# lucidrains/vit-pytorch

Hardware: NVIDIA H100
Metric: images/sec ViT-B/16 224^2 bf16 fwd (higher is better)
Workload: dtype bf16

## Files before the change

### vit_pytorch_b200/build.py

```python
from __future__ import annotations

import concurrent.futures as cf
import os
import shutil
import subprocess
import sys
from pathlib import Path

PKG = Path(__file__).resolve().parent
CSRC = PKG / "csrc"
LIBDIR = PKG / "lib"
OBJDIR = PKG / "lib" / "obj"
LIB = LIBDIR / "libb200vit.so"

NVCC_FLAGS = [
    "-gencode", "arch=compute_90a,code=sm_90a",
    "-std=c++17", "-O3", "-lineinfo",
    "-Xcompiler", "-fPIC",
    "--expt-relaxed-constexpr",
]


def _nvcc() -> str:
    nvcc = shutil.which("nvcc") or "/usr/local/cuda/bin/nvcc"
    if not os.path.exists(nvcc):
        raise RuntimeError("nvcc not found; libb200vit.so must be prebuilt in-tree")
    return nvcc


def sources() -> list[Path]:
    return sorted(CSRC.glob("*.cu"))


def needs_build() -> bool:
    if not LIB.exists():
        return True
    t = LIB.stat().st_mtime
    deps = list(CSRC.glob("*.cu")) + list(CSRC.glob("*.cuh")) + list(CSRC.glob("*.h")) + \
        [PKG.parent / "include" / "b200vit.h"]
    return any(d.stat().st_mtime > t for d in deps)


def _compile(src: Path, verbose: bool) -> Path:
    obj = OBJDIR / (src.stem + ".o")
    cmd = [_nvcc(), *NVCC_FLAGS, "-c", str(src), "-o", str(obj)]
    if verbose:
        cmd.insert(1, "-Xptxas")
        cmd.insert(2, "-v")
    r = subprocess.run(cmd, capture_output=True, text=True)
    if r.returncode != 0:
        raise RuntimeError(f"nvcc failed for {src.name}:\n{r.stdout}\n{r.stderr}")
    if verbose:
        print(r.stderr)
    return obj


def build(force: bool = False, verbose: bool = False) -> Path:
    if not force and not needs_build():
        return LIB
    OBJDIR.mkdir(parents=True, exist_ok=True)
    srcs = sources()
    with cf.ThreadPoolExecutor(max_workers=min(8, len(srcs))) as ex:
        objs = list(ex.map(lambda s: _compile(s, verbose), srcs))
    cmd = [_nvcc(), "-shared", "-gencode", "arch=compute_90a,code=sm_90a", "-o", str(LIB), *map(str, objs)]
    r = subprocess.run(cmd, capture_output=True, text=True)
    if r.returncode != 0:
        raise RuntimeError(f"link failed:\n{r.stdout}\n{r.stderr}")
    return LIB


if __name__ == "__main__":
    p = build(force="--force" in sys.argv, verbose="-v" in sys.argv)
    print(p)
```

### vit_pytorch_b200/csrc/gemm.cu

```cuda
#include "common.cuh"
#include "host_util.h"

namespace b200 {

constexpr int BLOCK_M = 128;
constexpr int BLOCK_K = 64;
constexpr int WGMMA_K = 16;
constexpr int NUM_THREADS = 384;
constexpr int NUM_CONSUMERS = 256;

struct GemmParams {
  int M, N, K;
  int num_m_tiles, num_n_tiles, num_k_blocks;
  int flags;
  __nv_bfloat16* out_bf16;
  float* out_f32;
  long long ldo;
  const float* bias;
  const float* ln_sums;
  int ln_parts;
  int stats_parts;
  int stats_width;
  float ln_inv_dim;
  float ln_eps;
  const float* col_s;
  float* stats_out;
  int rows_per_tile;
  int patch;
  int patch_ght;
  int patch_tiles_per_img;
  int patch_C;
};

template <int BLOCK_N, int STAGES, bool PATCH = false, bool RES = false, bool TMA_OUT = false>
struct GemmSmem {
  static constexpr bool BIAS_ONLY = RES && TMA_OUT && BLOCK_N == 256;
  static constexpr bool RING_SLABS = BIAS_ONLY;
  static constexpr int BUF_SLABS = RING_SLABS ? 0 : BLOCK_N / 64;
  static constexpr int A_SLAB = PATCH ? BLOCK_M * 32 : BLOCK_M * BLOCK_K * 2;
  static constexpr int A_BYTES = PATCH ? 4 * A_SLAB : A_SLAB;
  static constexpr int B_BYTES = BLOCK_N * BLOCK_K * 2;
  static constexpr int STAGE_BYTES = A_BYTES + B_BYTES;
  static constexpr int RES_BOX = BLOCK_M * 32 * 4;
  static constexpr int RES_SLAB = 2 * RES_BOX;
  static constexpr int RES_OFFSET = STAGES * STAGE_BYTES;
  static constexpr int OUT_BOX = 64 * 64 * 2;
  static constexpr int OUT_OFFSET = RES_OFFSET + (RES && !RING_SLABS ? 2 * RES_SLAB : 0);
  static constexpr int OUT_BYTES = !TMA_OUT ? 0 : RES ? 2 * OUT_BOX : BLOCK_M * BLOCK_N * 2;
  static constexpr int VEC_OFFSET = OUT_OFFSET + OUT_BYTES;
  static constexpr int VEC_BYTES = (BIAS_ONLY ? BLOCK_N : 2 * BLOCK_N + 2 * BLOCK_M) * 4;
  static constexpr int VEC_BUFS = BIAS_ONLY ? 1 : 2;
  static constexpr int BAR_OFFSET = VEC_OFFSET + VEC_BUFS * VEC_BYTES;
  static constexpr int TOTAL = BAR_OFFSET + (2 * STAGES + 8) * 8;
  static constexpr int DYN_BYTES = TOTAL + 1024;
};

__device__ __forceinline__ void warpgroup_sync(int c) { asm volatile("bar.sync %0, 128;" ::"r"(c + 1) : "memory"); }

template <int BLOCK_N, int STAGES, bool PATCH, bool RES, bool TMA_OUT, bool SIG = false, int EPI = -1>
__global__ void __launch_bounds__(NUM_THREADS, 1)
gemm_bf16_kernel(const __grid_constant__ CUtensorMap tmA, const __grid_constant__ CUtensorMap tmB,
                 const __grid_constant__ CUtensorMap tmR, const __grid_constant__ CUtensorMap tmO,
                 const __grid_constant__ CUtensorMap tmF, const GemmParams p) {
  static_assert(!(TMA_OUT && PATCH), "patch tiles have fewer than 128 rows: a 64-row box would overwrite the next one");
  static_assert(EPI < 0 || (TMA_OUT && !SIG), "compiled flag sets are for the TMA-store epilogue");
  using L = GemmSmem<BLOCK_N, STAGES, PATCH, RES, TMA_OUT>;
  constexpr int NACC = BLOCK_N / 2;
  constexpr int CHUNKS = BLOCK_N / 64;

  extern __shared__ uint8_t smem_raw[];
  uint8_t* smem = smem_raw + ((1024u - (smem_u32(smem_raw) & 1023u)) & 1023u);
  uint64_t* full_bar = reinterpret_cast<uint64_t*>(smem + L::BAR_OFFSET);
  uint64_t* empty_bar = full_bar + STAGES;
  uint64_t* res_full = empty_bar + STAGES;
  uint64_t* res_empty = res_full + 2;
  uint64_t* vec_full = res_empty + 2;
  uint64_t* vec_empty = vec_full + 2;

  const int wg = threadIdx.x >> 7;
  const int num_tiles = p.num_m_tiles * p.num_n_tiles;

  if (threadIdx.x == 0) {
    tma_prefetch_desc(&tmA);
    tma_prefetch_desc(&tmB);
    if (RES) tma_prefetch_desc(&tmR);
    if (TMA_OUT && p.out_bf16) tma_prefetch_desc(&tmO);
    if (TMA_OUT && RES && p.out_f32) tma_prefetch_desc(&tmF);
    for (int s = 0; s < STAGES; ++s) {
      mbar_init(&full_bar[s], 1);
      mbar_init(&empty_bar[s], 2);
    }
    for (int s = 0; s < 2; ++s) {
      mbar_init(&res_full[s], 1);
      mbar_init(&res_empty[s], TMA_OUT ? 2 : NUM_CONSUMERS);
      mbar_init(&vec_full[s], 64);
      mbar_init(&vec_empty[s], NUM_CONSUMERS);
    }
    fence_mbar_init();
  }
  __syncthreads();

  if (wg == 0) {
    setmaxnreg_dec<40>();
    if (threadIdx.x == 0) {
      int stage = 0;
      uint32_t phase = 0;
      for (int tile = blockIdx.x; tile < num_tiles; tile += gridDim.x) {
        const int m_blk = tile / p.num_n_tiles;
        const int n_blk = tile % p.num_n_tiles;
        for (int kb = 0; kb < p.num_k_blocks; ++kb) {
          mbar_wait(&empty_bar[stage], phase ^ 1);
          uint8_t* sa = smem + stage * L::STAGE_BYTES;
          uint8_t* sb = sa + L::A_BYTES;
          if (PATCH) {
            const int img = m_blk / p.patch_tiles_per_img, tin = m_blk % p.patch_tiles_per_img;
            mbar_arrive_expect_tx(&full_bar[stage], p.rows_per_tile * 128 + L::B_BYTES);
#pragma unroll
            for (int j = 0; j < 4; ++j)
              tma_load_5d(sa + j * L::A_SLAB, &tmA, &full_bar[stage], 0, 0, tin * p.patch_ght, (kb & 3) * 4 + j,
                          img * p.patch_C + (kb >> 2));
          } else {
            mbar_arrive_expect_tx(&full_bar[stage], L::STAGE_BYTES);
            tma_load_2d(sa, &tmA, &full_bar[stage], kb * BLOCK_K, m_blk * BLOCK_M);
          }
          tma_load_2d(sb, &tmB, &full_bar[stage], kb * BLOCK_K, n_blk * BLOCK_N);
          if (++stage == STAGES) {
            stage = 0;
            phase ^= 1;
          }
        }
        if (L::RING_SLABS) {
          const int n0 = n_blk * BLOCK_N;
          const int nslab = min(BLOCK_N / 64, (p.N - n0 + 63) / 64);
          for (int q = L::BUF_SLABS; q < nslab; ++q) {
            mbar_wait(&empty_bar[stage], phase ^ 1);
            const int c0 = n0 + 64 * q;
            const int nbox = c0 + 32 < p.N ? 2 : 1;
            mbar_arrive_expect_tx(&full_bar[stage], nbox * L::RES_BOX);
            uint8_t* slab = smem + stage * L::STAGE_BYTES;
            for (int b = 0; b < nbox; ++b)
              tma_load_2d(slab + b * L::RES_BOX, &tmR, &full_bar[stage], c0 + 32 * b, m_blk * BLOCK_M);
            if (++stage == STAGES) {
              stage = 0;
              phase ^= 1;
            }
          }
        }
      }
    } else if (RES && threadIdx.x == 32) {
      int it = 0;
      for (int tile = blockIdx.x; tile < num_tiles; tile += gridDim.x) {
        const int n0 = (tile % p.num_n_tiles) * BLOCK_N;
        const int m0 = (tile / p.num_n_tiles) * BLOCK_M;
        const int nslab = min(L::BUF_SLABS, (p.N - n0 + 63) / 64);
        for (int q = 0; q < nslab; ++q, ++it) {
          const int buf = it & 1;
          mbar_wait(&res_empty[buf], ((it >> 1) & 1) ^ 1);
          const int c0 = n0 + 64 * q;
          const int nbox = c0 + 32 < p.N ? 2 : 1;
          mbar_arrive_expect_tx(&res_full[buf], nbox * L::RES_BOX);
          uint8_t* slab = smem + L::RES_OFFSET + buf * L::RES_SLAB;
          for (int b = 0; b < nbox; ++b) tma_load_2d(slab + b * L::RES_BOX, &tmR, &res_full[buf], c0 + 32 * b, m0);
        }
      }
    } else if ((threadIdx.x >> 5) >= 2) {
      const int lane = threadIdx.x & 31;
      const bool vec_warp = (threadIdx.x >> 5) == 2;
      int it = 0;
      for (int tile = blockIdx.x; tile < num_tiles; tile += gridDim.x, ++it) {
        const int m_blk = tile / p.num_n_tiles;
        const int n0 = (tile % p.num_n_tiles) * BLOCK_N;
        const int vb = it % L::VEC_BUFS;
        mbar_wait(&vec_empty[vb], ((it / L::VEC_BUFS) & 1) ^ 1);
        float* vbias = reinterpret_cast<float*>(smem + L::VEC_OFFSET + vb * L::VEC_BYTES);
        float* vcs = vbias + BLOCK_N;
        float2* vln = reinterpret_cast<float2*>(vcs + BLOCK_N);
        if (vec_warp) {
#pragma unroll
          for (int i = lane; i < BLOCK_N; i += 32) {
            const int col = n0 + i;
            vbias[i] = (p.flags & B200VIT_EPI_BIAS) && col < p.N ? p.bias[col] : 0.f;
            if (!L::BIAS_ONLY) vcs[i] = (p.flags & B200VIT_EPI_LNFOLD) && col < p.N ? p.col_s[col] : 0.f;
          }
        } else if (!L::BIAS_ONLY && (p.flags & B200VIT_EPI_LNFOLD)) {
          float s1[BLOCK_M / 32], s2[BLOCK_M / 32];
          bool ok[BLOCK_M / 32];
#pragma unroll
          for (int k = 0; k < BLOCK_M / 32; ++k) {
            const int tr = lane + 32 * k;
            ok[k] = m_blk * p.rows_per_tile + tr < p.M && tr < p.rows_per_tile;
            s1[k] = s2[k] = 0.f;
          }
#pragma unroll 1
          for (int i = 0; i < p.ln_parts; ++i)
#pragma unroll
            for (int k = 0; k < BLOCK_M / 32; ++k)
              if (ok[k]) {
                const size_t row = (size_t)m_blk * p.rows_per_tile + lane + 32 * k;
                const float2 ss = *reinterpret_cast<const float2*>(p.ln_sums + 2 * (row * p.ln_parts + i));
                s1[k] += ss.x;
                s2[k] += ss.y;
              }
#pragma unroll
          for (int k = 0; k < BLOCK_M / 32; ++k) vln[lane + 32 * k] = make_float2(s1[k], s2[k]);
        }
        mbar_arrive(&vec_full[vb]);
      }
    }
    return;
  }

  setmaxnreg_inc<232>();
  const int c = wg - 1;
  const int t = threadIdx.x & 127;
  const int warp = t >> 5, lane = t & 31;
  const int flags = EPI >= 0 ? EPI : L::BIAS_ONLY ? p.flags & ~B200VIT_EPI_LNFOLD : p.flags;
  const bool vec_ok = (p.ldo & 1) == 0;
  int stage = 0;
  uint32_t phase = 0;
  int slab_it = 0;
  int pend_slab = -1;
  uint8_t* const stg_wg = smem + L::OUT_OFFSET + c * (RES ? L::OUT_BOX : 64 * BLOCK_N * 2);
  float acc[NACC];

  for (int tile = blockIdx.x, it = 0; tile < num_tiles; tile += gridDim.x, ++it) {
    const int m_blk = tile / p.num_n_tiles;
    const int n_blk = tile % p.num_n_tiles;

    int prev_stage = -1;
    for (int kb = 0; kb < p.num_k_blocks; ++kb) {
      mbar_wait(&full_bar[stage], phase);
      const uint32_t sa = smem_u32(smem + stage * L::STAGE_BYTES);
      const uint32_t sb = sa + L::A_BYTES;
      const uint64_t bdesc = make_wgmma_desc(sb, 1024, WGMMA_SW128);
      wgmma_fence();
#pragma unroll
      for (int k = 0; k < BLOCK_K / WGMMA_K; ++k) {
        const uint64_t ad = PATCH ? make_wgmma_desc(sa + k * L::A_SLAB + c * 64 * 32, 256, WGMMA_SW32)
                                  : make_wgmma_desc(sa + c * 64 * 128, 1024, WGMMA_SW128) + 2 * k;
        if constexpr (BLOCK_N == 256) wgmma_m64n256k16(acc, ad, bdesc + 2 * k, (kb | k) != 0);
        else wgmma_m64n128k16(acc, ad, bdesc + 2 * k, (kb | k) != 0);
      }
      wgmma_commit();
      if (TMA_OUT && kb == 0 && t == 0) {
        tma_store_wait_read<0>();
        if (RES && pend_slab >= 0) mbar_arrive(&empty_bar[pend_slab]);
        pend_slab = -1;
      }
      wgmma_wait<1>();
      if (prev_stage >= 0 && t == 0) mbar_arrive(&empty_bar[prev_stage]);
      prev_stage = stage;
      if (++stage == STAGES) {
        stage = 0;
        phase ^= 1;
      }
    }
    wgmma_wait<0>();
    fence_regs(acc);
    if (t == 0) mbar_arrive(&empty_bar[prev_stage]);
    if (TMA_OUT && !RES) warpgroup_sync(c);

    const int tr0 = c * 64 + warp * 16 + (lane >> 2);
    const int vb = it % L::VEC_BUFS;
    mbar_wait(&vec_full[vb], (it / L::VEC_BUFS) & 1);
    const float* vbias = reinterpret_cast<const float*>(smem + L::VEC_OFFSET + vb * L::VEC_BYTES);
    const float* vcs = vbias + BLOCK_N;
    const float2* vln = reinterpret_cast<const float2*>(vcs + BLOCK_N);
    float mu[2] = {0.f, 0.f}, rstd[2] = {1.f, 1.f};
    int row[2];
    bool row_ok[2];
#pragma unroll
    for (int h = 0; h < 2; ++h) {
      const int tr = tr0 + 8 * h;
      row[h] = m_blk * p.rows_per_tile + tr;
      row_ok[h] = row[h] < p.M && tr < p.rows_per_tile;
      if ((flags & B200VIT_EPI_LNFOLD) && row_ok[h]) {
        const float2 ss = vln[tr];
        const float s1 = ss.x, s2 = ss.y;
        mu[h] = s1 * p.ln_inv_dim;
        const float var = fmaxf(s2 * p.ln_inv_dim - mu[h] * mu[h], 0.f);
        rstd[h] = rsqrtf(var + p.ln_eps);
      }
    }
    float st_sum[2][CHUNKS], st_sq[2][CHUNKS];
#pragma unroll
    for (int q = 0; q < CHUNKS; ++q) st_sum[0][q] = st_sum[1][q] = st_sq[0][q] = st_sq[1][q] = 0.f;

    const int n0 = n_blk * BLOCK_N;
    const int nslab = RES ? min(CHUNKS, (p.N - n0 + 63) / 64) : 0;
    const int res_off = tr0 * 128 + (lane & 1) * 8;
    const int res_xor = ((lane & 3) >> 1) ^ (lane >> 2);
    const int stg_off = (tr0 - 64 * c) * 128 + 4 * (lane & 3);
    constexpr bool GUARD = EPI < 0 || RES;
#pragma unroll
    for (int j = 0; j < BLOCK_N / 8; ++j) {
      const int pc = 8 * j + 2 * (lane & 3);
      const int col = n0 + pc;
      const bool ring_slab = L::RING_SLABS && j / 8 >= L::BUF_SLABS;
      if (RES && j % 8 == 0 && j / 8 < nslab) {
        if (ring_slab) mbar_wait(&full_bar[stage], phase);
        else mbar_wait(&res_full[slab_it & 1], (slab_it >> 1) & 1);
      }
      uint8_t* const slab_base =
          smem + (ring_slab ? stage * L::STAGE_BYTES : L::RES_OFFSET + (slab_it & 1) * L::RES_SLAB);
      uint8_t* slab = slab_base + ((j % 8) / 4) * L::RES_BOX + res_off;
      uint8_t* stg = stg_wg + (RES ? 0 : (j / 8) * L::OUT_BOX) + stg_off + (((j % 8) ^ (lane >> 2)) << 4);
      const bool pair = vec_ok && col + 1 < p.N;
      float b0 = 0.f, b1 = 0.f, s0 = 0.f, s1 = 0.f;
      if (flags & B200VIT_EPI_BIAS) {
        const float2 bb = *reinterpret_cast<const float2*>(vbias + pc);
        b0 = bb.x;
        b1 = bb.y;
      }
      if (flags & B200VIT_EPI_LNFOLD) {
        const float2 ss = *reinterpret_cast<const float2*>(vcs + pc);
        s0 = ss.x;
        s1 = ss.y;
      }
#pragma unroll
      for (int h = 0; h < 2; ++h) {
        if (GUARD && (!row_ok[h] || col >= p.N)) continue;
        float v0 = acc[4 * j + 2 * h], v1 = acc[4 * j + 2 * h + 1];
        if (flags & (B200VIT_EPI_LNFOLD | B200VIT_EPI_BIAS)) {
          const bool fold = (flags & B200VIT_EPI_LNFOLD) != 0;
          const float k = -rstd[h] * mu[h];
          const float c0 = fold ? fmaf(k, s0, b0) : b0, c1 = fold ? fmaf(k, s1, b1) : b1;
          const float rs = fold ? rstd[h] : 1.0f;
          v0 = fmaf(v0, rs, c0);
          v1 = fmaf(v1, rs, c1);
        }
        if (flags & B200VIT_EPI_GELU) gelu_erf2(v0, v1);
        if (flags & B200VIT_EPI_HARDSWISH) {
          v0 = v0 * fminf(fmaxf(v0 + 3.0f, 0.0f), 6.0f) * (1.0f / 6.0f);
          v1 = v1 * fminf(fmaxf(v1 + 3.0f, 0.0f), 6.0f) * (1.0f / 6.0f);
        }
        if (SIG && (flags & (B200VIT_EPI_SILU | B200VIT_EPI_SIGMOID))) {
          const float g0 = fast_rcp(1.0f + fast_ex2(-1.4426950408889634f * v0));
          const float g1 = fast_rcp(1.0f + fast_ex2(-1.4426950408889634f * v1));
          const bool silu = (flags & B200VIT_EPI_SILU) != 0;
          v0 = silu ? v0 * g0 : g0;
          v1 = silu ? v1 * g1 : g1;
        }
        const size_t o = (size_t)row[h] * p.ldo + col;
        float2* rp = reinterpret_cast<float2*>(slab + h * 8 * 128 + ((((j % 4) * 2) ^ res_xor) << 4));
        float2 rr = make_float2(0.f, 0.f);
        if (RES) rr = *rp;
        float r0 = 0.f, r1 = 0.f;
        if (TMA_OUT) {
          if (RES) {
            v0 += rr.x;
            v1 += rr.y;
            *rp = make_float2(v0, v1);
          }
          const uint32_t pk = pack_bf16x2(v0, v1);
          if (!RES) *reinterpret_cast<uint32_t*>(stg + h * 8 * 128) = pk;
          r0 = __uint_as_float(pk << 16);
          r1 = __uint_as_float(pk & 0xFFFF0000u);
        } else if (pair) {
          if (RES) {
            v0 += rr.x;
            v1 += rr.y;
          }
          if (p.out_f32) *reinterpret_cast<float2*>(p.out_f32 + o) = make_float2(v0, v1);
          const uint32_t pk = pack_bf16x2(v0, v1);
          if (p.out_bf16) *reinterpret_cast<uint32_t*>(p.out_bf16 + o) = pk;
          r0 = __uint_as_float(pk << 16);
          r1 = __uint_as_float(pk & 0xFFFF0000u);
        } else {
          const float vv[2] = {v0, v1}, res[2] = {rr.x, rr.y};
          float rb[2] = {0.f, 0.f};
          for (int i = 0; i < 2 && col + i < p.N; ++i) {
            float x = vv[i];
            if (RES) x += res[i];
            if (p.out_f32) p.out_f32[o + i] = x;
            const __nv_bfloat16 xb = __float2bfloat16_rn(x);
            if (p.out_bf16) p.out_bf16[o + i] = xb;
            rb[i] = __bfloat162float(xb);
          }
          r0 = rb[0];
          r1 = rb[1];
        }
        if (flags & B200VIT_EPI_STATS) {
          st_sum[h][j / 8] += r0 + r1;
          st_sq[h][j / 8] = fmaf(r0, r0, fmaf(r1, r1, st_sq[h][j / 8]));
        }
      }
      if (RES && j % 8 == 7 && j / 8 < nslab) {
        if constexpr (TMA_OUT) {
          if (t == 0) {
            tma_store_wait_read<0>();
            if (pend_slab >= 0) mbar_arrive(&empty_bar[pend_slab]);
            pend_slab = -1;
          }
          warpgroup_sync(c);
          if (p.out_bf16)
#pragma unroll
            for (int jj = 0; jj < 8; ++jj)
#pragma unroll
              for (int h = 0; h < 2; ++h) {
                const float2 s = *reinterpret_cast<const float2*>(slab_base + (jj / 4) * L::RES_BOX + res_off +
                                                                  h * 8 * 128 + ((((jj % 4) * 2) ^ res_xor) << 4));
                *reinterpret_cast<uint32_t*>(stg_wg + stg_off + ((jj ^ (lane >> 2)) << 4) + h * 8 * 128) =
                    pack_bf16x2(s.x, s.y);
              }
          fence_proxy_async_smem();
          warpgroup_sync(c);
          if (t == 0) {
            const int c0 = n0 + 64 * (j / 8), row0 = m_blk * BLOCK_M + 64 * c;
            if (row0 < p.M) {
              const uint8_t* half = slab_base + c * 64 * 128;
              if (p.out_f32)
                for (int b = 0; b < 2 && c0 + 32 * b < p.N; ++b)
                  tma_store_2d(&tmF, half + b * L::RES_BOX, c0 + 32 * b, row0);
              if (p.out_bf16) tma_store_2d(&tmO, stg_wg, c0, row0);
            }
            tma_store_commit();
            pend_slab = ring_slab ? stage : STAGES + 2 + (slab_it & 1);
          }
        } else {
          mbar_arrive(&res_empty[slab_it & 1]);
        }
        if (ring_slab) {
          if (++stage == STAGES) {
            stage = 0;
            phase ^= 1;
          }
        } else {
          ++slab_it;
        }
      }
    }
    mbar_arrive(&vec_empty[vb]);
    if constexpr (TMA_OUT && !RES) {
      fence_proxy_async_smem();
      warpgroup_sync(c);
      if (t == 0) {
        const int row0 = m_blk * BLOCK_M + 64 * c;
        if (row0 < p.M)
          for (int b = 0; b < BLOCK_N / 64 && n0 + 64 * b < p.N; ++b)
            tma_store_2d(&tmO, stg_wg + b * L::OUT_BOX, n0 + 64 * b, row0);
        tma_store_commit();
      }
    }
    if (flags & B200VIT_EPI_STATS) {
#pragma unroll
      for (int h = 0; h < 2; ++h)
#pragma unroll
        for (int q = 0; q < CHUNKS; ++q) {
          st_sum[h][q] += __shfl_xor_sync(0xffffffffu, st_sum[h][q], 1);
          st_sum[h][q] += __shfl_xor_sync(0xffffffffu, st_sum[h][q], 2);
          st_sq[h][q] += __shfl_xor_sync(0xffffffffu, st_sq[h][q], 1);
          st_sq[h][q] += __shfl_xor_sync(0xffffffffu, st_sq[h][q], 2);
        }
      if ((lane & 3) == 0) {
        const int per = p.stats_width / 64;
        const int first = n0 / p.stats_width;
        const int last = (n_blk == p.num_n_tiles - 1) ? p.stats_parts : first + CHUNKS / per;
#pragma unroll
        for (int h = 0; h < 2; ++h) {
          if (!row_ok[h]) continue;
          float* so = p.stats_out + 2 * (size_t)(row[0] + 8 * h) * p.stats_parts;
          for (int part = first; part < last; ++part) {
            float a = 0.f, b = 0.f;
#pragma unroll
            for (int q = 0; q < CHUNKS; ++q)
              if (first + q / per == part) {
                a += st_sum[h][q];
                b += st_sq[h][q];
              }
            *reinterpret_cast<float2*>(so + 2 * part) = make_float2(a, b);
          }
        }
      }
    }
  }
  if (TMA_OUT && t == 0) tma_store_wait<0>();
}

static std::atomic<int> g_gemm_block_n{0};
void gemm_set_block_n(int v) { g_gemm_block_n = v; }
static std::atomic<int> g_gemm_direct_store{0};
void gemm_set_direct_store(int v) { g_gemm_direct_store = v; }

template <int BLOCK_N, int STAGES, bool PATCH = false, bool RES = false, bool TMA_OUT = false, bool SIG = false,
          int EPI = -1>
static int launch_gemm(const CUtensorMap& tmA, const CUtensorMap& tmB, const CUtensorMap& tmR, const CUtensorMap& tmO,
                       const CUtensorMap& tmF, GemmParams& p, cudaStream_t stream) {
  using L = GemmSmem<BLOCK_N, STAGES, PATCH, RES, TMA_OUT>;
  static_assert(L::DYN_BYTES <= 227 * 1024, "gemm: shared memory budget");
  static_assert(!L::BIAS_ONLY || L::DYN_BYTES == 215168, "gemm: 256 x 4 residual TMA-store layout changed");
  auto kern = gemm_bf16_kernel<BLOCK_N, STAGES, PATCH, RES, TMA_OUT, SIG, EPI>;
  B200_ENSURE_SMEM(kern, L::DYN_BYTES);
  if (!p.patch) p.rows_per_tile = BLOCK_M;
  p.num_m_tiles = (p.M + p.rows_per_tile - 1) / p.rows_per_tile;
  p.num_n_tiles = (p.N + BLOCK_N - 1) / BLOCK_N;
  p.num_k_blocks = (p.K + BLOCK_K - 1) / BLOCK_K;
  p.stats_width = p.N > 128 ? 128 : 64;
  const int tiles = p.num_m_tiles * p.num_n_tiles;
  const int grid = tiles < num_sms() ? tiles : num_sms();
  kern<<<grid, NUM_THREADS, L::DYN_BYTES, stream>>>(tmA, tmB, tmR, tmO, tmF, p);
  B200_CHECK_CUDA(cudaGetLastError());
  count_launch();
  return 0;
}

template <int BLOCK_N, int STAGES, bool RES>
static int launch_tma_out(const CUtensorMap& tmA, const CUtensorMap& tmB, const CUtensorMap& tmR,
                          const CUtensorMap& tmO, const CUtensorMap& tmF, GemmParams& p, cudaStream_t stream) {
  constexpr int QKV = B200VIT_EPI_BIAS | B200VIT_EPI_LNFOLD, FC1 = QKV | B200VIT_EPI_GELU;
  constexpr int RES_STATS = B200VIT_EPI_RESIDUAL | B200VIT_EPI_STATS, RES_STATS_BIAS = RES_STATS | B200VIT_EPI_BIAS;
  if constexpr (RES) {
    if (p.flags == RES_STATS_BIAS)
      return launch_gemm<BLOCK_N, STAGES, false, true, true, false, RES_STATS_BIAS>(tmA, tmB, tmR, tmO, tmF, p, stream);
    if (p.flags == RES_STATS)
      return launch_gemm<BLOCK_N, STAGES, false, true, true, false, RES_STATS>(tmA, tmB, tmR, tmO, tmF, p, stream);
  } else {
    if (p.flags == QKV)
      return launch_gemm<BLOCK_N, STAGES, false, false, true, false, QKV>(tmA, tmB, tmR, tmO, tmF, p, stream);
    if (p.flags == FC1)
      return launch_gemm<BLOCK_N, STAGES, false, false, true, false, FC1>(tmA, tmB, tmR, tmO, tmF, p, stream);
  }
  return launch_gemm<BLOCK_N, STAGES, false, RES, true>(tmA, tmB, tmR, tmO, tmF, p, stream);
}

}

extern "C" int b200vit_stats_parts(int N) {
  const int block_n = N > 128 ? 256 : 128;
  return 2 * ((N + block_n - 1) / block_n);
}

extern "C" int b200vit_gemm_bf16(const void* A, int64_t lda, const void* W, int64_t ldw, void* out_bf16,
                                 float* out_f32, int64_t ldo, const float* bias, const float* resid,
                                 const float* ln_sums, int ln_parts, float ln_eps, const float* col_s,
                                 float* stats_out, int M, int N, int K, int flags, void* stream) {
  using namespace b200;
  B200_CHECK_ARG(A && W, "gemm: A/W must not be null");
  B200_CHECK_ARG(out_bf16 || out_f32, "gemm: need at least one output");
  B200_CHECK_ARG(M > 0 && N > 0 && K > 0, "gemm: bad shape M=%d N=%d K=%d", M, N, K);
  B200_CHECK_ARG((reinterpret_cast<uintptr_t>(A) & 15) == 0 && (reinterpret_cast<uintptr_t>(W) & 15) == 0,
                 "gemm: A and W must be 16-byte aligned");
  B200_CHECK_ARG((lda & 7) == 0 && (ldw & 7) == 0 && lda >= K && ldw >= K,
                 "gemm: lda=%lld ldw=%lld must be multiples of 8 and >= K=%d", (long long)lda, (long long)ldw, K);
  B200_CHECK_ARG(ldo >= N, "gemm: ldo=%lld < N=%d", (long long)ldo, N);
  B200_CHECK_ARG(!(flags & B200VIT_EPI_BIAS) || bias, "gemm: EPI_BIAS without bias");
  B200_CHECK_ARG(!(flags & B200VIT_EPI_RESIDUAL) || resid, "gemm: EPI_RESIDUAL without resid");
  B200_CHECK_ARG(!(flags & B200VIT_EPI_RESIDUAL) || (ldo & 3) == 0,
                 "gemm: EPI_RESIDUAL needs ldo=%lld to be a multiple of 4 (16-byte rows for TMA)", (long long)ldo);
  B200_CHECK_ARG(!(flags & B200VIT_EPI_LNFOLD) || (ln_sums && col_s && ln_parts >= 1 && ln_parts <= 64),
                 "gemm: EPI_LNFOLD needs ln_sums, col_s and 1 <= ln_parts <= 64");
  B200_CHECK_ARG(!(flags & B200VIT_EPI_STATS) || stats_out, "gemm: EPI_STATS without stats_out");
  B200_CHECK_ARG(!(flags & B200VIT_EPI_RESIDUAL) || !(flags & (B200VIT_EPI_SILU | B200VIT_EPI_SIGMOID)),
                 "gemm: EPI_SILU and EPI_SIGMOID do not combine with EPI_RESIDUAL");
  const int act = flags & (B200VIT_EPI_GELU | B200VIT_EPI_HARDSWISH | B200VIT_EPI_SILU | B200VIT_EPI_SIGMOID);
  B200_CHECK_ARG((act & (act - 1)) == 0,
                 "gemm: EPI_GELU, EPI_HARDSWISH, EPI_SILU and EPI_SIGMOID are exclusive (flags 0x%x)", flags);
  auto al16 = [](const void* q) { return (reinterpret_cast<uintptr_t>(q) & 15) == 0; };
  B200_CHECK_ARG(al16(bias) && al16(resid) && al16(col_s) && al16(out_bf16) && al16(out_f32) && al16(ln_sums),
                 "gemm: epilogue pointers must be 16-byte aligned");

  cudaStream_t st = reinterpret_cast<cudaStream_t>(stream);

  GemmParams p{};
  p.M = M; p.N = N; p.K = K;
  p.flags = flags;
  p.out_bf16 = reinterpret_cast<__nv_bfloat16*>(out_bf16);
  p.out_f32 = out_f32;
  p.ldo = ldo;
  p.bias = bias;
  p.ln_sums = ln_sums;
  p.ln_parts = ln_parts;
  p.stats_parts = b200vit_stats_parts(N);
  p.ln_inv_dim = 1.0f / (float)K;
  p.ln_eps = ln_eps;
  p.col_s = col_s;
  p.stats_out = stats_out;

  const bool res = (flags & B200VIT_EPI_RESIDUAL) != 0;
  const bool tma_ok = !g_gemm_direct_store.load() && ((ldo | N) & 7) == 0 && (res || !out_f32);
  const bool lnfold = (flags & B200VIT_EPI_LNFOLD) != 0;
  const int force = g_gemm_block_n.load();
  const bool res_wide_pays = (long long)((M + BLOCK_M - 1) / BLOCK_M) * ((N + 255) / 256) >= num_sms();
  const bool sig = (flags & (B200VIT_EPI_SILU | B200VIT_EPI_SIGMOID)) != 0;
  const bool wide = !sig && (force == 0 ? N > 128 && (!(res && tma_ok) || (!lnfold && res_wide_pays)) : force == 2);
  const uint32_t block_n = wide ? 256 : 128;
  const bool tma_out = tma_ok && !(res && wide && lnfold);
  CUtensorMap tmA, tmB, tmR{}, tmO{}, tmF{};
  if (tma_out && out_bf16) {
    const uint64_t dims[2] = {(uint64_t)N, (uint64_t)M};
    const uint64_t strides[1] = {(uint64_t)ldo * 2};
    const uint32_t box[2] = {64, 64};
    int rc = encode_tmap_bf16(&tmO, out_bf16, 2, dims, strides, box);
    if (rc) return rc;
  }
  if (tma_out && res && out_f32) {
    const uint64_t dims[2] = {(uint64_t)N, (uint64_t)M};
    const uint64_t strides[1] = {(uint64_t)ldo * 4};
    const uint32_t box[2] = {32, 64};
    int rc = encode_tmap_f32(&tmF, out_f32, 2, dims, strides, box, true);
    if (rc) return rc;
  }
  if (res) {
    const uint64_t dims[2] = {(uint64_t)N, (uint64_t)M};
    const uint64_t strides[1] = {(uint64_t)ldo * 4};
    const uint32_t box[2] = {32, (uint32_t)BLOCK_M};
    int rc = encode_tmap_f32(&tmR, resid, 2, dims, strides, box, true);
    if (rc) return rc;
  }
  {
    const uint64_t dims[2] = {(uint64_t)K, (uint64_t)M};
    const uint64_t strides[1] = {(uint64_t)lda * 2};
    const uint32_t box[2] = {(uint32_t)BLOCK_K, (uint32_t)BLOCK_M};
    int rc = encode_tmap_bf16(&tmA, A, 2, dims, strides, box);
    if (rc) return rc;
  }
  {
    const uint64_t dims[2] = {(uint64_t)K, (uint64_t)N};
    const uint64_t strides[1] = {(uint64_t)ldw * 2};
    const uint32_t box[2] = {(uint32_t)BLOCK_K, block_n};
    int rc = encode_tmap_bf16(&tmB, W, 2, dims, strides, box);
    if (rc) return rc;
  }
  if (sig)
    return tma_out ? launch_gemm<128, 5, false, false, true, true>(tmA, tmB, tmR, tmO, tmF, p, st)
                   : launch_gemm<128, 6, false, false, false, true>(tmA, tmB, tmR, tmO, tmF, p, st);
  if (tma_out) {
    if (res)
      return wide ? launch_tma_out<256, 4, true>(tmA, tmB, tmR, tmO, tmF, p, st)
                  : launch_tma_out<128, 4, true>(tmA, tmB, tmR, tmO, tmF, p, st);
    return wide ? launch_tma_out<256, 3, false>(tmA, tmB, tmR, tmO, tmF, p, st)
                : launch_tma_out<128, 5, false>(tmA, tmB, tmR, tmO, tmF, p, st);
  }
  if (wide)
    return res ? launch_gemm<256, 3, false, true>(tmA, tmB, tmR, tmO, tmF, p, st)
               : launch_gemm<256, 4>(tmA, tmB, tmR, tmO, tmF, p, st);
  return res ? launch_gemm<128, 4, false, true>(tmA, tmB, tmR, tmO, tmF, p, st)
             : launch_gemm<128, 6>(tmA, tmB, tmR, tmO, tmF, p, st);
}

extern "C" int b200vit_rmsnorm_heads(void* buf, int64_t ld, const float* gamma, int T, int nheads, int dh, void* stream);
extern "C" int b200vit_layernorm_heads(void* buf, int64_t ld, const float* gamma, int T, int nheads, int dh, float eps,
                                       void* stream);

extern "C" int b200vit_gemm_headnorm_bf16(const void* A, int64_t lda, const void* W, int64_t ldw, void* out_bf16,
                                          int64_t ldo, const float* bias, const float* ln_sums, int ln_parts,
                                          float ln_eps, const float* col_s, const float* head_gamma, int norm_heads,
                                          int dh, float head_eps, int M, int N, int K, int flags, void* stream) {
  using namespace b200;
  B200_CHECK_ARG(out_bf16 && head_gamma, "gemm_headnorm: null pointer");
  B200_CHECK_ARG(head_width_ok(dh), "gemm_headnorm: dim_head=%d not supported by this build (32, 64, 80 or 128)", dh);
  B200_CHECK_ARG(norm_heads > 0 && norm_heads * dh <= N, "gemm_headnorm: %d heads do not fit N=%d", norm_heads, N);
  B200_CHECK_ARG((flags & ~(B200VIT_EPI_BIAS | B200VIT_EPI_LNFOLD | B200VIT_EPI_HEADLN)) == 0,
                 "gemm_headnorm: unsupported flags %d", flags);
  const bool hln = (flags & B200VIT_EPI_HEADLN) != 0;
  B200_CHECK_ARG((reinterpret_cast<uintptr_t>(head_gamma) & 15) == 0, "gemm_headnorm: head_gamma must be 16-byte aligned");
  int rc = b200vit_gemm_bf16(A, lda, W, ldw, out_bf16, nullptr, ldo, bias, nullptr, ln_sums, ln_parts, ln_eps, col_s,
                             nullptr, M, N, K, flags & ~B200VIT_EPI_HEADLN, stream);
  if (rc) return rc;
  if (hln) return b200vit_layernorm_heads(out_bf16, ldo, head_gamma, M, norm_heads, dh, head_eps, stream);
  return b200vit_rmsnorm_heads(out_bf16, ldo, head_gamma, M, norm_heads, dh, stream);
}


extern "C" int b200vit_patch_embed_tma(const void* img, const void* w_perm, const float* bias, const float* col_s,
                                       const float* patch_stats, float ln_eps, float* out_f32, int64_t ldo, int B, int C,
                                       int H, int W, int D, void* stream) {
  using namespace b200;
  B200_CHECK_ARG(img && w_perm && bias && col_s && patch_stats && out_f32, "patch_embed_tma: null pointer");
  B200_CHECK_ARG(B > 0 && C > 0 && C <= 8 && H > 0 && W > 0 && (H % 16) == 0 && (W % 16) == 0,
                 "patch_embed_tma: needs 16 x 16 patches on an image whose sides are multiples of 16 (got %dx%d)", H, W);
  B200_CHECK_ARG(D > 0 && (D % 8) == 0 && ldo >= D, "patch_embed_tma: bad D=%d / ldo", D);
  B200_CHECK_ARG((reinterpret_cast<uintptr_t>(img) & 15) == 0 && (reinterpret_cast<uintptr_t>(w_perm) & 15) == 0 &&
                     (reinterpret_cast<uintptr_t>(out_f32) & 15) == 0 && (reinterpret_cast<uintptr_t>(bias) & 15) == 0 &&
                     (reinterpret_cast<uintptr_t>(col_s) & 15) == 0,
                 "patch_embed_tma: pointers must be 16-byte aligned");
  const int gh = H / 16, gw = W / 16;
  B200_CHECK_ARG(gw <= 128, "patch_embed_tma: %d patches per row do not fit a 128-row tile", gw);
  int ght = 1;
  for (int d = 1; d <= gh; ++d)
    if (gh % d == 0 && d * gw <= 128) ght = d;
  const int K = C * 256;
  GemmParams p{};
  p.M = B * gh * gw; p.N = D; p.K = K;
  p.flags = B200VIT_EPI_LNFOLD | B200VIT_EPI_BIAS;
  p.out_f32 = out_f32;
  p.ldo = ldo;
  p.bias = bias;
  p.ln_sums = patch_stats;
  p.ln_parts = 1;
  p.stats_parts = b200vit_stats_parts(D);
  p.ln_inv_dim = 1.0f / (float)K;
  p.ln_eps = ln_eps;
  p.col_s = col_s;
  p.patch = 1;
  p.patch_ght = ght;
  p.patch_tiles_per_img = gh / ght;
  p.patch_C = C;
  p.rows_per_tile = ght * gw;
  CUtensorMap tmA, tmB, tmR{}, tmO{}, tmF{};
  {
    const uint64_t dims[5] = {16, (uint64_t)gw, (uint64_t)gh, 16, (uint64_t)B * C};
    const uint64_t strides[4] = {32, (uint64_t)16 * W * 2, (uint64_t)W * 2, (uint64_t)H * W * 2};
    const uint32_t box[5] = {16, (uint32_t)gw, (uint32_t)ght, 1, 1};
    int rc = encode_tmap_bf16_sw(&tmA, img, 5, dims, strides, box, 32);
    if (rc) return rc;
  }
  {
    const uint64_t dims[2] = {(uint64_t)K, (uint64_t)D};
    const uint64_t strides[1] = {(uint64_t)K * 2};
    const uint32_t box[2] = {(uint32_t)BLOCK_K, 256};
    int rc = encode_tmap_bf16(&tmB, w_perm, 2, dims, strides, box);
    if (rc) return rc;
  }
  return launch_gemm<256, 4, true>(tmA, tmB, tmR, tmO, tmF, p, reinterpret_cast<cudaStream_t>(stream));
}
```

Baseline: 13580.

## Defer accumulator drain past epilogue setup and prefetch bias/scale vectors

Moves the final wgmma wait, stage release and TMA-store read wait in the GEMM consumer from right after the K loop to after the per-tile vector and LayerNorm-statistics setup, so that setup overlaps in-flight MMAs. For non-residual TMA-store outputs, the wait on the previous tile's store is also moved from the first K iteration to just before staging. A small register read-ahead of bias and column-scale pairs is added to the epilogue for the fused QKV/FC1 variants. A separately built phase-timing library with clock64 instrumentation is added, but it is compiled out of the default library.

```diff
diff --git a/vit_pytorch_b200/build.py b/vit_pytorch_b200/build.py
--- a/vit_pytorch_b200/build.py
+++ b/vit_pytorch_b200/build.py
@@ -12,6 +12,8 @@
 LIBDIR = PKG / "lib"
 OBJDIR = PKG / "lib" / "obj"
 LIB = LIBDIR / "libb200vit.so"
+PHASES_LIB = LIBDIR / "libb200vit_phases.so"
+PHASES_SRC = "gemm.cu"
 
 NVCC_FLAGS = [
     "-gencode", "arch=compute_90a,code=sm_90a",
@@ -33,17 +35,17 @@
 
 
 def needs_build() -> bool:
-    if not LIB.exists():
+    if not LIB.exists() or not PHASES_LIB.exists():
         return True
-    t = LIB.stat().st_mtime
+    t = min(LIB.stat().st_mtime, PHASES_LIB.stat().st_mtime)
     deps = list(CSRC.glob("*.cu")) + list(CSRC.glob("*.cuh")) + list(CSRC.glob("*.h")) + \
         [PKG.parent / "include" / "b200vit.h"]
     return any(d.stat().st_mtime > t for d in deps)
 
 
-def _compile(src: Path, verbose: bool) -> Path:
-    obj = OBJDIR / (src.stem + ".o")
-    cmd = [_nvcc(), *NVCC_FLAGS, "-c", str(src), "-o", str(obj)]
+def _compile(src: Path, verbose: bool, phases: bool = False) -> Path:
+    obj = OBJDIR / (src.stem + ("_phases.o" if phases else ".o"))
+    cmd = [_nvcc(), *NVCC_FLAGS, *(["-DB200VIT_GEMM_PHASES"] if phases else []), "-c", str(src), "-o", str(obj)]
     if verbose:
         cmd.insert(1, "-Xptxas")
         cmd.insert(2, "-v")
@@ -60,13 +62,20 @@
         return LIB
     OBJDIR.mkdir(parents=True, exist_ok=True)
     srcs = sources()
-    with cf.ThreadPoolExecutor(max_workers=min(8, len(srcs))) as ex:
-        objs = list(ex.map(lambda s: _compile(s, verbose), srcs))
-    cmd = [_nvcc(), "-shared", "-gencode", "arch=compute_90a,code=sm_90a", "-o", str(LIB), *map(str, objs)]
+    jobs = [(s, False) for s in srcs] + [(CSRC / PHASES_SRC, True)]
+    with cf.ThreadPoolExecutor(max_workers=min(8, len(jobs))) as ex:
+        objs = list(ex.map(lambda j: _compile(j[0], verbose, j[1]), jobs))
+    phases_obj = objs.pop()
+    _link(LIB, objs)
+    _link(PHASES_LIB, [phases_obj if o.name == Path(PHASES_SRC).stem + ".o" else o for o in objs])
+    return LIB
+
+
+def _link(lib: Path, objs: list[Path]) -> None:
+    cmd = [_nvcc(), "-shared", "-gencode", "arch=compute_90a,code=sm_90a", "-o", str(lib), *map(str, objs)]
     r = subprocess.run(cmd, capture_output=True, text=True)
     if r.returncode != 0:
-        raise RuntimeError(f"link failed:\n{r.stdout}\n{r.stderr}")
-    return LIB
+        raise RuntimeError(f"link of {lib.name} failed:\n{r.stdout}\n{r.stderr}")
 
 
 if __name__ == "__main__":
diff --git a/vit_pytorch_b200/csrc/gemm.cu b/vit_pytorch_b200/csrc/gemm.cu
--- a/vit_pytorch_b200/csrc/gemm.cu
+++ b/vit_pytorch_b200/csrc/gemm.cu
@@ -8,6 +8,17 @@
 constexpr int WGMMA_K = 16;
 constexpr int NUM_THREADS = 384;
 constexpr int NUM_CONSUMERS = 256;
+
+#ifdef B200VIT_GEMM_PHASES
+#define GEMM_PHASE(...) __VA_ARGS__
+enum : int { PH_START, PH_FIRST_FULL, PH_STORE_WAIT, PH_LAST_ISSUE, PH_DRAINED, PH_VEC, PH_STAGED, PH_COMMITTED,
+             PH_FULL_WAIT, PH_CONS };
+enum : int { PH_EMPTY_WAIT, PH_EMPTY_WAIT0, PH_LN_START, PH_LN_END, PH_LOAD };
+enum : int { PH_CLK0, PH_GT0, PH_CLK1, PH_GT1, PH_SMID, PH_CTA };
+constexpr int PH_TILE = 2 * PH_CONS + PH_LOAD;
+#else
+#define GEMM_PHASE(...)
+#endif
 
 struct GemmParams {
   int M, N, K;
@@ -30,6 +41,9 @@
   int patch_ght;
   int patch_tiles_per_img;
   int patch_C;
+#ifdef B200VIT_GEMM_PHASES
+  long long* phases;
+#endif
 };
 
 template <int BLOCK_N, int STAGES, bool PATCH = false, bool RES = false, bool TMA_OUT = false>
@@ -108,8 +122,12 @@
       for (int tile = blockIdx.x; tile < num_tiles; tile += gridDim.x) {
         const int m_blk = tile / p.num_n_tiles;
         const int n_blk = tile % p.num_n_tiles;
+        GEMM_PHASE(long long* ph = p.phases ? p.phases + (size_t)tile * PH_TILE + 2 * PH_CONS : nullptr;
+                   long long empty_wait = 0;)
         for (int kb = 0; kb < p.num_k_blocks; ++kb) {
+          GEMM_PHASE(const long long w0 = clock64();)
           mbar_wait(&empty_bar[stage], phase ^ 1);
+          GEMM_PHASE(const long long w = clock64() - w0; empty_wait += w; if (ph && kb == 0) ph[PH_EMPTY_WAIT0] = w;)
           uint8_t* sa = smem + stage * L::STAGE_BYTES;
           uint8_t* sb = sa + L::A_BYTES;
           if (PATCH) {
@@ -129,6 +147,7 @@
             phase ^= 1;
           }
         }
+        GEMM_PHASE(if (ph) ph[PH_EMPTY_WAIT] = empty_wait;)
         if (L::RING_SLABS) {
           const int n0 = n_blk * BLOCK_N;
           const int nslab = min(BLOCK_N / 64, (p.N - n0 + 63) / 64);
@@ -183,6 +202,8 @@
             if (!L::BIAS_ONLY) vcs[i] = (p.flags & B200VIT_EPI_LNFOLD) && col < p.N ? p.col_s[col] : 0.f;
           }
         } else if (!L::BIAS_ONLY && (p.flags & B200VIT_EPI_LNFOLD)) {
+          GEMM_PHASE(long long* ph = p.phases && lane == 0 ? p.phases + (size_t)tile * PH_TILE + 2 * PH_CONS : nullptr;
+                     if (ph) ph[PH_LN_START] = clock64();)
           float s1[BLOCK_M / 32], s2[BLOCK_M / 32];
           bool ok[BLOCK_M / 32];
 #pragma unroll
@@ -203,6 +224,7 @@
               }
 #pragma unroll
           for (int k = 0; k < BLOCK_M / 32; ++k) vln[lane + 32 * k] = make_float2(s1[k], s2[k]);
+          GEMM_PHASE(if (ph) ph[PH_LN_END] = clock64();)
         }
         mbar_arrive(&vec_full[vb]);
       }
@@ -222,14 +244,27 @@
   int pend_slab = -1;
   uint8_t* const stg_wg = smem + L::OUT_OFFSET + c * (RES ? L::OUT_BOX : 64 * BLOCK_N * 2);
   float acc[NACC];
+  GEMM_PHASE(long long* const ph_cta =
+                 p.phases && c == 0 && t == 0 ? p.phases + (size_t)num_tiles * PH_TILE + blockIdx.x * PH_CTA : nullptr;
+             if (ph_cta) {
+               ph_cta[PH_CLK0] = clock64();
+               ph_cta[PH_GT0] = globaltimer_ns();
+             })
 
   for (int tile = blockIdx.x, it = 0; tile < num_tiles; tile += gridDim.x, ++it) {
     const int m_blk = tile / p.num_n_tiles;
     const int n_blk = tile % p.num_n_tiles;
+    GEMM_PHASE(long long* const ph = p.phases && t == 0 ? p.phases + (size_t)tile * PH_TILE + c * PH_CONS : nullptr;
+               long long full_wait = 0; if (ph) ph[PH_START] = clock64();)
 
     int prev_stage = -1;
     for (int kb = 0; kb < p.num_k_blocks; ++kb) {
+      GEMM_PHASE(const long long w0 = clock64();)
       mbar_wait(&full_bar[stage], phase);
+      GEMM_PHASE(if (ph) {
+        if (kb == 0) ph[PH_FIRST_FULL] = clock64();
+        else full_wait += clock64() - w0;
+      })
       const uint32_t sa = smem_u32(smem + stage * L::STAGE_BYTES);
       const uint32_t sb = sa + L::A_BYTES;
       const uint64_t bdesc = make_wgmma_desc(sb, 1024, WGMMA_SW128);
@@ -242,9 +277,12 @@
         else wgmma_m64n128k16(acc, ad, bdesc + 2 * k, (kb | k) != 0);
       }
       wgmma_commit();
-      if (TMA_OUT && kb == 0 && t == 0) {
+      GEMM_PHASE(if (ph && kb == p.num_k_blocks - 1) ph[PH_LAST_ISSUE] = clock64();)
+      if (TMA_OUT && RES && kb == 0 && t == 0) {
+        GEMM_PHASE(const long long s0 = clock64();)
         tma_store_wait_read<0>();
-        if (RES && pend_slab >= 0) mbar_arrive(&empty_bar[pend_slab]);
+        GEMM_PHASE(if (ph) ph[PH_STORE_WAIT] = clock64() - s0;)
+        if (pend_slab >= 0) mbar_arrive(&empty_bar[pend_slab]);
         pend_slab = -1;
       }
       wgmma_wait<1>();
@@ -255,14 +293,10 @@
         phase ^= 1;
       }
     }
-    wgmma_wait<0>();
-    fence_regs(acc);
-    if (t == 0) mbar_arrive(&empty_bar[prev_stage]);
-    if (TMA_OUT && !RES) warpgroup_sync(c);
-
     const int tr0 = c * 64 + warp * 16 + (lane >> 2);
     const int vb = it % L::VEC_BUFS;
     mbar_wait(&vec_full[vb], (it / L::VEC_BUFS) & 1);
+    GEMM_PHASE(if (ph) ph[PH_VEC] = clock64();)
     const float* vbias = reinterpret_cast<const float*>(smem + L::VEC_OFFSET + vb * L::VEC_BYTES);
     const float* vcs = vbias + BLOCK_N;
     const float2* vln = reinterpret_cast<const float2*>(vcs + BLOCK_N);
@@ -282,6 +316,22 @@
         rstd[h] = rsqrtf(var + p.ln_eps);
       }
     }
+    wgmma_wait<0>();
+    fence_regs(acc);
+    GEMM_PHASE(if (ph) {
+      ph[PH_DRAINED] = clock64();
+      ph[PH_FULL_WAIT] = full_wait;
+    })
+    if (t == 0) mbar_arrive(&empty_bar[prev_stage]);
+    if (TMA_OUT && !RES) {
+      if (t == 0) {
+        GEMM_PHASE(const long long s0 = clock64();)
+        tma_store_wait_read<0>();
+        GEMM_PHASE(if (ph) ph[PH_STORE_WAIT] = clock64() - s0;)
+      }
+      warpgroup_sync(c);
+    }
+
     float st_sum[2][CHUNKS], st_sq[2][CHUNKS];
 #pragma unroll
     for (int q = 0; q < CHUNKS; ++q) st_sum[0][q] = st_sum[1][q] = st_sq[0][q] = st_sq[1][q] = 0.f;
@@ -292,10 +342,24 @@
     const int res_xor = ((lane & 3) >> 1) ^ (lane >> 2);
     const int stg_off = (tr0 - 64 * c) * 128 + 4 * (lane & 3);
     constexpr bool GUARD = EPI < 0 || RES;
+    constexpr bool VEC_AHEAD = TMA_OUT && !RES && EPI >= 0;
+    constexpr int VEC_AHEAD_GROUPS = 2;
+    float2 ahead_b[VEC_AHEAD_GROUPS], ahead_s[VEC_AHEAD_GROUPS];
+    auto read_ahead = [&](int j) {
+      const int slot = j % VEC_AHEAD_GROUPS, pc = 8 * j + 2 * (lane & 3);
+      if (flags & B200VIT_EPI_BIAS) ahead_b[slot] = *reinterpret_cast<const float2*>(vbias + pc);
+      if (flags & B200VIT_EPI_LNFOLD) ahead_s[slot] = *reinterpret_cast<const float2*>(vcs + pc);
+    };
+    if (VEC_AHEAD)
+#pragma unroll
+      for (int j = 0; j < VEC_AHEAD_GROUPS; ++j) read_ahead(j);
 #pragma unroll
     for (int j = 0; j < BLOCK_N / 8; ++j) {
       const int pc = 8 * j + 2 * (lane & 3);
       const int col = n0 + pc;
+      const float2 vec_b = VEC_AHEAD ? ahead_b[j % VEC_AHEAD_GROUPS] : float2{},
+                   vec_s = VEC_AHEAD ? ahead_s[j % VEC_AHEAD_GROUPS] : float2{};
+      if (VEC_AHEAD && j + VEC_AHEAD_GROUPS < BLOCK_N / 8) read_ahead(j + VEC_AHEAD_GROUPS);
       const bool ring_slab = L::RING_SLABS && j / 8 >= L::BUF_SLABS;
       if (RES && j % 8 == 0 && j / 8 < nslab) {
         if (ring_slab) mbar_wait(&full_bar[stage], phase);
@@ -308,12 +372,12 @@
       const bool pair = vec_ok && col + 1 < p.N;
       float b0 = 0.f, b1 = 0.f, s0 = 0.f, s1 = 0.f;
       if (flags & B200VIT_EPI_BIAS) {
-        const float2 bb = *reinterpret_cast<const float2*>(vbias + pc);
+        const float2 bb = VEC_AHEAD ? vec_b : *reinterpret_cast<const float2*>(vbias + pc);
         b0 = bb.x;
         b1 = bb.y;
       }
       if (flags & B200VIT_EPI_LNFOLD) {
-        const float2 ss = *reinterpret_cast<const float2*>(vcs + pc);
+        const float2 ss = VEC_AHEAD ? vec_s : *reinterpret_cast<const float2*>(vcs + pc);
         s0 = ss.x;
         s1 = ss.y;
       }
@@ -434,6 +498,7 @@
     if constexpr (TMA_OUT && !RES) {
       fence_proxy_async_smem();
       warpgroup_sync(c);
+      GEMM_PHASE(if (ph) ph[PH_STAGED] = clock64();)
       if (t == 0) {
         const int row0 = m_blk * BLOCK_M + 64 * c;
         if (row0 < p.M)
@@ -441,6 +506,9 @@
             tma_store_2d(&tmO, stg_wg + b * L::OUT_BOX, n0 + 64 * b, row0);
         tma_store_commit();
       }
+      GEMM_PHASE(if (ph) ph[PH_COMMITTED] = clock64();)
+    } else {
+      GEMM_PHASE(if (ph) ph[PH_STAGED] = ph[PH_COMMITTED] = clock64();)
     }
     if (flags & B200VIT_EPI_STATS) {
 #pragma unroll
@@ -475,12 +543,23 @@
     }
   }
   if (TMA_OUT && t == 0) tma_store_wait<0>();
+  GEMM_PHASE(if (ph_cta) {
+    uint32_t smid;
+    asm volatile("mov.u32 %0, %%smid;" : "=r"(smid));
+    ph_cta[PH_CLK1] = clock64();
+    ph_cta[PH_GT1] = globaltimer_ns();
+    ph_cta[PH_SMID] = smid;
+  })
 }
 
 static std::atomic<int> g_gemm_block_n{0};
 void gemm_set_block_n(int v) { g_gemm_block_n = v; }
 static std::atomic<int> g_gemm_direct_store{0};
 void gemm_set_direct_store(int v) { g_gemm_direct_store = v; }
+#ifdef B200VIT_GEMM_PHASES
+static std::atomic<long long*> g_gemm_phases{nullptr};
+static std::atomic<long long> g_gemm_phase_slots{0};
+#endif
 
 template <int BLOCK_N, int STAGES, bool PATCH = false, bool RES = false, bool TMA_OUT = false, bool SIG = false,
           int EPI = -1>
@@ -498,6 +577,8 @@
   p.stats_width = p.N > 128 ? 128 : 64;
   const int tiles = p.num_m_tiles * p.num_n_tiles;
   const int grid = tiles < num_sms() ? tiles : num_sms();
+  GEMM_PHASE(p.phases = (long long)tiles * PH_TILE + (long long)grid * PH_CTA <= g_gemm_phase_slots.load()
+                            ? g_gemm_phases.load() : nullptr;)
   kern<<<grid, NUM_THREADS, L::DYN_BYTES, stream>>>(tmA, tmB, tmR, tmO, tmF, p);
   B200_CHECK_CUDA(cudaGetLastError());
   count_launch();
@@ -524,6 +605,14 @@
 }
 
 }
+
+#ifdef B200VIT_GEMM_PHASES
+extern "C" void b200vit_gemm_phases(long long* buf, long long slots) {
+  b200::g_gemm_phase_slots = 0;
+  b200::g_gemm_phases = buf;
+  b200::g_gemm_phase_slots = buf ? slots : 0;
+}
+#endif
 
 extern "C" int b200vit_stats_parts(int N) {
   const int block_n = N > 128 ? 256 : 128;
```

New measurement: 13960 (median of 6 runs). 1.03x the previous value.
